# watsonyanghx/GAN_Lib_Tensorflow

Measured on AMD Instinct MI355X. Metric: images/sec (G+D step) SNGAN-ResNet CIFAR-10 bs=64, higher is better.
Workload: dtype bf16; 1 GPU; SNGAN ResNet CIFAR-10 32x32 bs=64 hinge: 1 G update (2x64 fakes) + 5 D updates (64 real + 64 fake) per step; global_batch=64, per_gpu_batch=64, parallelism=dp1, graphs=True, finite=True, collectives_in_graphs=False, grad_wire=fp32

## Files before the change

gan_lib_tensorflow_amd/csrc/conv_igemm.hip:

```cpp
#include "gank_common.h"
#ifdef GANK_TUNING
static __device__ int gank_stats_dbg = 0;
static void gank_stats_dbg_init() {
  static const int v = gank_tune("GANK_STATS_DBG", 0);
  static bool done = false;
  if (!done) { done = true; if (v) (void)hipMemcpyToSymbol(HIP_SYMBOL(gank_stats_dbg), &v, sizeof(int)); }
}
#else
static inline void gank_stats_dbg_init() {}
#endif
#include <stdlib.h>
#include <type_traits>

#ifndef GANK_KMODE
#define GANK_KMODE 0
#endif
#define IG_IN_ZEROINS2X 16
#define IG_IN_STRIDE2 32
#define IG_RES_UP2X 128

struct IgemmArgs {
  const bf16* x;
  const bf16* w;
  const float* bias;
// ... 686 lines not shown
    u32x4 v = {0u, 0u, 0u, 0u};
    if (row < a.Cout && row < 3) v = *reinterpret_cast<const u32x4*>(a.w + (long)row * a.Kpad + c8 * 8);
    *reinterpret_cast<u32x4*>(sW + row * wrow + c8 * 8) = v;
  }

  int h_off[6], h_lds[6];
#pragma unroll
  for (int j = 0; j < 6; j++) {
    const int q = tid + NT * j;
    const int hp = q >> 3, cc = q & 7;
    const int iy = py0 - 1 + hp / 18, ix = px0 - 1 + hp % 18;
    const bool ok = q < PHALO * 8 && (unsigned)iy < (unsigned)a.H && (unsigned)ix < (unsigned)a.W;
    h_off[j] = ok ? (((n * a.H + iy) * a.W + ix) * a.Cin + cc * 8) * 2 : OOB;
    h_lds[j] = (q < PHALO * 8) ? (hp / 18) * HROWP + (hp % 18) * LROW + cc * 8 : -1;
  }
  u32x4 rH[6];
  constexpr bool NORM = (MODE & 8) != 0;
  f32x4 nm[NORM ? 8 : 1];
  const float* np_mu = nullptr;
  const float* np_ga = nullptr;
  const float* np_be = nullptr;
  if constexpr (NORM) {
    int lb = a.cbn_labels[n];
    lb = lb < 0 ? 0 : (lb >= a.cbn_n_labels ? a.cbn_n_labels - 1 : lb);
    np_mu = a.cbn_stats + (long)(n / a.cbn_n_per_group) * 2 * a.Cin + (tid & 7) * 8;
    np_ga = a.cbn_gamma + (long)lb * a.Cin + (tid & 7) * 8;
    np_be = a.cbn_beta + (long)lb * a.Cin + (tid & 7) * 8;
  }
  auto load_halo = [&](int c) {
#pragma unroll
    for (int j = 0; j < 6; j++)
      rH[j] = __builtin_amdgcn_raw_buffer_load_b128(rs_x, h_off[j] == OOB ? OOB : h_off[j] + c * 128, 0, 0);
    if constexpr (NORM) {
      nm[0] = *reinterpret_cast<const f32x4*>(np_mu + c * 64); nm[1] = *reinterpret_cast<const f32x4*>(np_mu + c * 64 + 4);
      nm[2] = *reinterpret_cast<const f32x4*>(np_mu + a.Cin + c * 64); nm[3] = *reinterpret_cast<const f32x4*>(np_mu + a.Cin + c * 64 + 4);
      nm[4] = *reinterpret_cast<const f32x4*>(np_ga + c * 64); nm[5] = *reinterpret_cast<const f32x4*>(np_ga + c * 64 + 4);
      nm[6] = *reinterpret_cast<const f32x4*>(np_be + c * 64); nm[7] = *reinterpret_cast<const f32x4*>(np_be + c * 64 + 4);
    }
  };
  auto store_halo = [&]() {
#pragma unroll
    for (int j = 0; j < 6; j++) {
      if (h_lds[j] >= 0) {
        u32x4 v = rH[j];
        if constexpr (NORM) {
          if (h_off[j] != OOB) {
            const bf16x8 xv = __builtin_bit_cast(bf16x8, v);
            bf16x8 o;
#pragma unroll
            for (int e = 0; e < 8; e++) {
              const float mu = e < 4 ? nm[0][e] : nm[1][e - 4], iv = e < 4 ? nm[2][e] : nm[3][e - 4];
              const float ga = e < 4 ? nm[4][e] : nm[5][e - 4], be = e < 4 ? nm[6][e] : nm[7][e - 4];
              const float t = (bf2f(xv[e]) - mu) * iv * ga + be;
              o[e] = f2bf(fmaxf(t, 0.f));
            }
            v = __builtin_bit_cast(u32x4, o);
          }
        } else if constexpr ((MODE & 1) != 0) {
          v = relu_bf16x8(v);
        }
        *reinterpret_cast<u32x4*>(sP + h_lds[j]) = v;
      }
    }
  };

  f32x16 acc;
#pragma unroll
  for (int e = 0; e < 16; e++) acc[e] = 0.f;
  const int pb = (wave * 2 + (r >> 4) + 1) * HROWP + ((r & 15) + 1) * LROW + h * 8;
  const int ab = (r < 3 ? r : 3) * wrow + h * 8;

  const int nchunks = a.Cin >> 6;
  load_halo(0);
  store_halo();
  __syncthreads();
#pragma unroll 1
  for (int c = 0; c < nchunks; c++) {
    if (c + 1 < nchunks) load_halo(c + 1);
    const bf16* pW = sW + ab + c * 64;
#pragma unroll
    for (int tap = 0; tap < 9; tap++) {
      const int toff = (tap / 3 - 1) * HROWP + (tap % 3 - 1) * LROW;
#pragma unroll
      for (int kk = 0; kk < 4; kk++) {
        const bf16x8 fa = *reinterpret_cast<const bf16x8*>(pW + tap * a.Cin + kk * 16);
        const bf16x8 fb = *reinterpret_cast<const bf16x8*>(sP + pb + toff + kk * 16);
        acc = GANK_MFMA32(fa, fb, acc);
      }
    }
    if (c + 1 < nchunks) {
      __syncthreads();
      store_halo();
      __syncthreads();
    }
  }

  if (h == 0) {
    const bool otanh = (a.flags & GANK_OUT_TANH) != 0;
    const int py = wave * 2 + (r >> 4), px = r & 15;
    const long m = ((long)(n * a.H + py0 + py)) * a.W + px0 + px;
#pragma unroll
    for (int e = 0; e < 3; e++) {
      if (e >= a.Cout) break;
      float t = acc[e] * a.scale;
      if (a.bias) t += a.bias[e];
      if (a.mask) t = (bf2f(a.mask[m * a.Cout + e]) > 0.f) ? t : 0.f;
      if (a.res) t += bf2f(a.res[m * a.Cout + e]);
      a.y[m * a.Cout + e] = f2bf(otanh ? tanhf(t) : t);
    }
  }
}

template <int MODE>
static int launch_few(const IgemmArgs& a0, hipStream_t s) {
  IgemmArgs a = a0;
  a.tiles_m = a.N * (a.H / 8) * (a.W / 16);
  a.tiles_n = 1;
  const size_t lds = ((size_t)10 * HROWP + (size_t)4 * (a.Kpad + 8)) * sizeof(bf16);
  auto kern = conv3x3_few_kernel<MODE>;
  GANK_MAX_DYNAMIC_LDS(kern, (int)lds, "conv3x3_few");
  static const std::string tag = gank_format("conv3x3_few_kernel<%d>", MODE);
  gank_prof_tag(0, tag.c_str());
  hipLaunchKernelGGL(kern, dim3(a.tiles_m), dim3(256), lds, s, a);
  GANK_LAUNCH_OK("conv3x3_few");
  return 0;
}
static bool few_ok(const IgemmArgs& a) {
  static const int env = gank_tune("GANK_IGEMM_FEW", 1);
  return env && a.korder == 0 && a.Cout <= 3 && a.CoutPad == 32 && a.Cin % 64 == 0 && a.Kpad == 9 * a.Cin && !(a.flags & IG_RES_UP2X) &&
         (size_t)(10 * HROWP + 4 * (a.Kpad + 8)) * sizeof(bf16) <= 160 * 1024;
}

template <int MODE>
static int launch_patch_phase(const IgemmArgs& a0, hipStream_t s) {
  IgemmArgs a = a0;
  a.tiles_pp = a.N * (a.H / 8) * (a.W / 16);
  a.phase_inner = phase_inner_env();
  a.tiles_m = 4 * a.tiles_pp;
  a.tiles_n = a.CoutPad / 128;
  const size_t lds = ((size_t)10 * HROWP + (size_t)2 * 128 * LROW) * sizeof(bf16);
  auto kern = conv_igemm_patch_kernel<MODE, 128>;
  GANK_MAX_DYNAMIC_LDS(kern, (int)lds, "conv_igemm_patch");
  static const std::string tag = gank_format("conv_igemm_patch_kernel<%d, 128>", MODE);
  gank_prof_tag(0, tag.c_str());
  hipLaunchKernelGGL(kern, dim3(a.tiles_m * a.tiles_n), dim3(256), lds, s, a);
  GANK_LAUNCH_OK("conv_igemm_patch_phase");
  return 0;
}
static bool patch_phase_ok(const IgemmArgs& a) {
  static const int env = gank_tune("GANK_IGEMM_PATCH_PHASE", 1);
  return env && a.W % 16 == 0 && a.H % 8 == 0 && a.CoutPad % 128 == 0 && a.Cout % 4 == 0 && a.Cin % 64 == 0;
}

constexpr int NARROW_LDS = 4 * 32 * 272;
template <int KS, int CIN, bool POOL>
__device__ __forceinline__ void narrow_in_body(const IgemmArgs& a, const int block, char* s_t) {
  constexpr int TAPS = KS * KS, KTOT = TAPS * CIN, PAD = (KS - 1) / 2;
  static_assert(KTOT <= 32, "one 32-deep K-step");
  static_assert(!POOL || KS == 1, "pooled gather: 1x1 only");
  const int lane = threadIdx.x & 63, wave = threadIdx.x >> 6;
  const int r = lane & 31, h = lane >> 5;
  const int tile_n = block % a.tiles_n, tile_m = block / a.tiles_n;
  const int m = tile_m * 128 + wave * 32 + r;
  const bool inrelu = (a.flags & GANK_IN_RELU) != 0;

  int n = 0, oh = 0, ow = 0;
  if (m < a.M) pix_decomp(m, a.H, a.W, a.shw, a.sw, n, oh, ow);
  bf16x8 fb[2];
#pragma unroll
  for (int kk = 0; kk < 2; kk++) {
#pragma unroll
    for (int j = 0; j < 8; j++) {
      const int k = kk * 16 + 8 * h + j;
      const int tap = k / CIN, c = k - tap * CIN;
      const int ih = oh + tap / KS - PAD, iw = ow + tap % KS - PAD;
      const bool ok = m < a.M && k < KTOT && (unsigned)ih < (unsigned)a.H && (unsigned)iw < (unsigned)a.W;
      float val;
      if constexpr (POOL) {
        const int rs = 2 * a.W * CIN;
        const int idx = ok ? ((n * 2 * a.H + 2 * ih) * 2 * a.W + 2 * iw) * CIN + c : 0;
        val = bf2f(f2bf((bf2f(a.x[idx]) + bf2f(a.x[idx + rs]) + bf2f(a.x[idx + CIN]) + bf2f(a.x[idx + rs + CIN])) * 0.25f));
      } else {
        const int idx = ok ? ((n * a.H + ih) * a.W + iw) * CIN + c : 0;
        val = bf2f(a.x[idx]);
      }
      val = ok ? val : 0.f;
      if (inrelu) val = fmaxf(val, 0.f);
      fb[kk][j] = f2bf(val);
    }
  }
  if constexpr (POOL) {
    if (a.aux_out && tile_n == 0 && h == 0 && m < a.M) {
#pragma unroll
      for (int j = 0; j < CIN; j++) a.aux_out[(long)m * CIN + j] = fb[0][j];
    }
  }
  f32x16 acc[4];
#pragma unroll
  for (int i = 0; i < 4; i++)
#pragma unroll
    for (int e = 0; e < 16; e++) acc[i][e] = 0.f;
#pragma unroll
  for (int i = 0; i < 4; i++) {
    const bf16* wr = a.w + (long)(tile_n * 128 + i * 32 + r) * a.Kpad + h * 8;
#pragma unroll
    for (int kk = 0; kk < 2; kk++) {
      const bf16x8 fa = *reinterpret_cast<const bf16x8*>(wr + kk * 16);
      acc[i] = GANK_MFMA32(fa, fb[kk], acc[i]);
    }
  }
  const bool otanh = (a.flags & GANK_OUT_TANH) != 0;
  if (a.korder == 0 && !a.mask && !a.res && !otanh && (a.Cout & 127) == 0) {
    char* mine = s_t + wave * 32 * 272;
#pragma unroll
    for (int i = 0; i < 4; i++) {
      const int ct = tile_n * 128 + i * 32;
#pragma unroll
      for (int q = 0; q < 2; q++) {
        float v[8];
        acc_widen(acc[i], q, a.scale, v);
        bf16x8 o;
        if (a.bias) {
          const f32x4 b0 = *reinterpret_cast<const f32x4*>(a.bias + ct + 16 * q + 8 * h), b1 = *reinterpret_cast<const f32x4*>(a.bias + ct + 16 * q + 8 * h + 4);
#pragma unroll
          for (int e = 0; e < 4; e++) { v[e] += b0[e]; v[4 + e] += b1[e]; }
        }
#pragma unroll
        for (int e = 0; e < 8; e++) o[e] = f2bf(v[e]);
        *reinterpret_cast<bf16x8*>(mine + r * 272 + (i * 32 + 16 * q + 8 * h) * 2) = o;
      }
    }
    asm volatile("s_waitcnt lgkmcnt(0)" ::: "memory");
    const int m_w = tile_m * 128 + wave * 32;
#pragma unroll
    for (int it = 0; it < 8; it++) {
      const int p = it * 4 + (lane >> 4), c16 = lane & 15;
      const u32x4 v = *reinterpret_cast<const u32x4*>(mine + p * 272 + c16 * 16);
      if (m_w + p < a.M) *reinterpret_cast<u32x4*>(a.y + (long)(m_w + p) * a.Cout + tile_n * 128 + c16 * 8) = v;
    }
    return;
  }
  if ((a.Cout & 31) == 0) {
    if (m < a.M) {
#pragma unroll
      for (int i = 0; i < 4; i++) {
        const int ct = tile_n * 128 + i * 32;
        if (ct < a.Cout)
          epi_tile_wide<false>(acc[i], a.scale, a.bias ? a.bias + ct : nullptr, a.mask ? a.mask + (long)m * a.Cout + ct : nullptr,
                               a.res ? a.res + (long)m * a.Cout + ct : nullptr, a.y + (long)m * a.Cout + ct, h, otanh, nullptr);
      }
    }
    return;
  }
#pragma unroll
  for (int i = 0; i < 4; i++) {
    const int co0 = tile_n * 128 + i * 32 + 4 * h;
#pragma unroll
    for (int g = 0; g < 4; g++) {
      const int co = co0 + 8 * g;
      float v[4];
#pragma unroll
      for (int e = 0; e < 4; e++) v[e] = acc[i][4 * g + e] * a.scale;
      if (m < a.M && co < a.Cout) {
        const long o = (long)m * a.Cout + co;
        if (a.bias) {
          const f32x4 b = *reinterpret_cast<const f32x4*>(a.bias + co);
#pragma unroll
          for (int e = 0; e < 4; e++) v[e] += b[e];
        }
        if (a.mask) {
          const bf16x4 mk = *reinterpret_cast<const bf16x4*>(a.mask + o);
#pragma unroll
          for (int e = 0; e < 4; e++) v[e] = (bf2f(mk[e]) > 0.f) ? v[e] : 0.f;
        }
        if (a.res) {
          const bf16x4 rs = *reinterpret_cast<const bf16x4*>(a.res + o);
#pragma unroll
          for (int e = 0; e < 4; e++) v[e] += bf2f(rs[e]);
        }
        bf16x4 out;
#pragma unroll
        for (int e = 0; e < 4; e++) out[e] = f2bf(otanh ? tanhf(v[e]) : v[e]);
        *reinterpret_cast<bf16x4*>(a.y + o) = out;
      }
    }
  }
}

template <int KS, int CIN, bool POOL = false>
__global__ __launch_bounds__(256) void conv_narrow_in_kernel(IgemmArgs a) {
  __shared__ __attribute__((aligned(16))) char s_t[NARROW_LDS];
  narrow_in_body<KS, CIN, POOL>(a, blockIdx.x, s_t);
}
__global__ __launch_bounds__(256) void conv_narrow_in_pair_kernel(IgemmArgs a, IgemmArgs b, int blocks_a) {
  __shared__ __attribute__((aligned(16))) char s_t[NARROW_LDS];
  if ((int)blockIdx.x < blocks_a) narrow_in_body<3, 3, false>(a, blockIdx.x, s_t);
  else narrow_in_body<1, 3, true>(b, blockIdx.x - blocks_a, s_t);
}

template <int KS, int CIN, bool POOL = false>
static int launch_narrow_in(const IgemmArgs& a0, hipStream_t s) {
  IgemmArgs a = a0;
  a.tiles_m = cdiv(a.M, 128);
  a.tiles_n = a.CoutPad / 128;
  static const std::string tag = gank_format("conv_narrow_in_kernel<%d, %d%s>", KS, CIN, POOL ? ", pool" : "");
  gank_prof_tag(0, tag.c_str());
  hipLaunchKernelGGL((conv_narrow_in_kernel<KS, CIN, POOL>), dim3(a.tiles_m * a.tiles_n), dim3(256), 0, s, a);
  GANK_LAUNCH_OK("conv_narrow_in");
  return 0;
}

constexpr int PP_HALO_BYTES = 24576;
constexpr int PP_WSLOT_BYTES = 16384;
constexpr int PP_NSLOT = 6, PP_PD = 4;
constexpr int PP_WRING = 2 * PP_HALO_BYTES;
constexpr int PP_LDS_BYTES = PP_WRING + PP_NSLOT * PP_WSLOT_BYTES;

template <int N>
__device__ __forceinline__ void pp_wait_vmcnt() {
  static_assert(N == 0 || N == 4 || N == 6 || N == 7, "vmcnt value not instantiated");
  if constexpr (N == 0) asm volatile("s_waitcnt vmcnt(0)" ::: "memory");
  if constexpr (N == 4) asm volatile("s_waitcnt vmcnt(4)" ::: "memory");
  if constexpr (N == 6) asm volatile("s_waitcnt vmcnt(6)" ::: "memory");
  if constexpr (N == 7) asm volatile("s_waitcnt vmcnt(7)" ::: "memory");
}

#ifndef GANK_PP_M16
#define GANK_PP_M16 1
#endif
#ifdef GANK_ACT_F16
#define GANK_MFMA16(a, b, c) __builtin_amdgcn_mfma_f32_16x16x32_f16(a, b, c, 0, 0, 0)
#else
#define GANK_MFMA16(a, b, c) __builtin_amdgcn_mfma_f32_16x16x32_bf16(a, b, c, 0, 0, 0)
#endif
template <int MODE, int PW, bool STATS = false>
__global__ __launch_bounds__(512) void conv_igemm_pp_kernel(IgemmArgs a) {
  constexpr bool PHASE = (MODE & 4) != 0;
  constexpr int NT = PHASE ? 4 : 9;
  constexpr int PHH = 256 / PW;
  constexpr int HW_ = PW + 2, HROW = HW_ * 64;
  constexpr int HPX = (PHH + 2) * HW_;
  constexpr int RS = 32 / PW;
  constexpr int HSW = PW == 16 ? 1 : 2;
#if GANK_PP_M16
  auto pp_hswz = [](int hx) { return (hx >> 1) & 2; };
  auto pp_wswz = [](int co) { return (co >> 1) & 2; };
#else
  auto pp_hswz = [](int hx) { return (hx >> HSW) & 3; };
  auto pp_wswz = [](int co) { return (co >> 2) & 3; };
#endif
  static_assert(PW == 32 || PW == 16, "patch width");
  static_assert(HPX * 64 <= PP_HALO_BYTES, "halo image");
  extern __shared__ __attribute__((aligned(16))) char smem[];
  typedef __attribute__((address_space(3))) void* lds_t;
  const int tid = threadIdx.x, lane = tid & 63;
  const int wave = __builtin_amdgcn_readfirstlane(tid >> 6);
  const int wm = wave >> 2, wn = wave & 3;
  const int r = lane & 31, h = lane >> 5;
  const int prow = RS == 1 ? 0 : (r >> 4), pcol = RS == 1 ? r : (r & 15);

  const int nwg = a.tiles_m * a.tiles_n;
  const int lid = xcd_remap(blockIdx.x, nwg);
  const int tile_n = lid % a.tiles_n;
  int tile_m = lid / a.tiles_n;
  int phase = 0;
  if constexpr (PHASE) {
    if (a.phase_inner) { phase = tile_m & 3; tile_m >>= 2; }
    else { phase = tile_m / a.tiles_pp; tile_m -= phase * a.tiles_pp; }
  }
  const int pad_h = PHASE ? 1 - (phase >> 1) : 1, pad_w = PHASE ? 1 - (phase & 1) : 1;
  const int pw = a.W / PW, ph = a.H / PHH;
  const int n = tile_m / (pw * ph), pr = tile_m - n * pw * ph;
  const int py0 = (pr / pw) * PHH, px0 = (pr % pw) * PW;

  constexpr unsigned OOB = 0x7FFFFFF0u;
  const __amdgpu_buffer_rsrc_t rs_x = __builtin_amdgcn_make_buffer_rsrc(const_cast<bf16*>(a.x), 0, a.N * a.H * a.W * a.Cin * 2, 0x00020000);
  const __amdgpu_buffer_rsrc_t rs_w = __builtin_amdgcn_make_buffer_rsrc(const_cast<bf16*>(a.w) + (PHASE ? (long)phase * a.CoutPad * a.Kpad : 0L), 0,
                                                                        a.CoutPad * a.Kpad * 2, 0x00020000);

  unsigned h_off[6];
#pragma unroll
  for (int j = 0; j < 6; j++) {
    const int q = (j * 4 + wn) * 64 + lane;
    const int hp = q >> 2, hy = hp / HW_, hx = hp - hy * HW_;
    const int iy = py0 - 1 + hy, ix = px0 - 1 + hx;
    const bool ok = hp < HPX && (unsigned)iy < (unsigned)a.H && (unsigned)ix < (unsigned)a.W;
    h_off[j] = ok ? (unsigned)((((n * a.H + iy) * a.W + ix) * a.Cin + (((q & 3) ^ pp_hswz(hx)) << 3)) * 2) : OOB;
  }
  int w_off[2];
#pragma unroll
  for (int j = 0; j < 2; j++) {
    const int q = (j * 8 + wave) * 64 + lane;
    const int co = q >> 2;
    w_off[j] = ((tile_n * 256 + co) * a.Kpad + (((q & 3) ^ pp_wswz(co)) << 3)) * 2;
  }
  constexpr int ND = PHASE ? 2 : 3;
#if GANK_PP_M16
  const int p16 = lane & 15, kc = lane >> 4;
  constexpr int RPT = PW / 16;
  int a_lane, b_lane[ND];
  a_lane = PP_WRING + (wn * 64 + p16) * 64 + ((kc ^ pp_wswz(p16)) << 4);
#pragma unroll
  for (int d = 0; d < ND; d++) {
    const int hx = p16 + d + (PHASE ? 1 - pad_w : 0);
    const int hy = wm * (PHH / 2) + (PHASE ? 1 - pad_h : 0);
    b_lane[d] = hy * HROW + hx * 64 + ((kc ^ pp_hswz(hx)) << 4);
  }
#else
  int a_lane[2], b_lane[ND][2];
#pragma unroll
  for (int kk = 0; kk < 2; kk++) {
    a_lane[kk] = PP_WRING + (wn * 64 + r) * 64 + (((kk * 2 + h) ^ pp_wswz(r)) << 4);
#pragma unroll
    for (int d = 0; d < ND; d++) {
      const int hx = pcol + d + (PHASE ? 1 - pad_w : 0);
      const int hy = wm * (PHH / 2) + prow + (PHASE ? 1 - pad_h : 0);
      b_lane[d][kk] = hy * HROW + hx * 64 + (((kk * 2 + h) ^ pp_hswz(hx)) << 4);
    }
  }
#endif

  const int nch = a.Cin >> 5;
  auto issue_w = [&](int slot_bytes, int c, int tap) {
    const int koff = (tap * a.Cin + c * 32) * 2;
#pragma unroll
    for (int j = 0; j < 2; j++)
      __builtin_amdgcn_raw_ptr_buffer_load_lds(rs_w, (lds_t)(smem + PP_WRING + slot_bytes + (j * 8 + wave) * 1024), 16, w_off[j], koff, 0, 0);
  };
  auto issue_h = [&](int buf, int c, int j0) {
#pragma unroll
    for (int j = j0; j < j0 + 3; j++)
      __builtin_amdgcn_raw_ptr_buffer_load_lds(rs_x, (lds_t)(smem + buf * PP_HALO_BYTES + (j * 4 + wn) * 1024), 16, (int)(h_off[j] + (unsigned)c * 64u), 0, 0, 0);
  };

#if GANK_PP_M16
  f32x4 acc[4][8];
#pragma unroll
  for (int i = 0; i < 4; i++)
#pragma unroll
    for (int j = 0; j < 8; j++) acc[i][j] = f32x4{0.f, 0.f, 0.f, 0.f};
#else
  f32x16 acc[2][4];
#pragma unroll
  for (int i = 0; i < 2; i++)
#pragma unroll
    for (int j = 0; j < 4; j++)
#pragma unroll
      for (int e = 0; e < 16; e++) acc[i][j][e] = 0.f;
#endif

  if (wm == 1) { issue_h(0, 0, 0); issue_h(0, 0, 3); }
  {
    int c = 0, t = 0;
#pragma unroll
    for (int q = 0; q < PP_PD; q++) {
      issue_w(q * PP_WSLOT_BYTES, c, t);
      if (++t == NT) { t = 0; c++; }
      if (c >= nch) { c = nch - 1; t = NT - 1; }
    }
  }
// ... 415 lines not shown
  const bool pp_ok = pp_env() && patch_geom && a.Cout % 256 == 0 && a.Kpad == a.taps * a.Cin && pp_enough_blocks(a, 1) &&
                     (pp_env() >= 2 || pp_patch_width(a.H, a.W) == 32);
  if (narrow_ok) {
    rc = a.ks == 3 ? launch_narrow_in<3, 3>(a, s) : launch_narrow_in<1, 3>(a, s);
  } else if (pp_ok) {
    const bool relu = (a.flags & GANK_IN_RELU) != 0;
    if (pp_patch_width(a.H, a.W) == 32) rc = relu ? launch_pp<1, 32>(a, s) : launch_pp<0, 32>(a, s);
    else rc = relu ? launch_pp<1, 16>(a, s) : launch_pp<0, 16>(a, s);
  } else if (patch_ok) {
    rc = (a.flags & GANK_IN_RELU) ? launch_patch<1, 128>(a, s) : launch_patch<0, 128>(a, s);
  } else if (patch32_ok && few_ok(a)) {
    rc = (a.flags & GANK_IN_RELU) ? launch_few<1>(a, s) : launch_few<0>(a, s);
  } else if (patch32_ok) {
    rc = (a.flags & GANK_IN_RELU) ? launch_patch<1, 32>(a, s) : launch_patch<0, 32>(a, s);
  } else if (packed) {
    if (a.CoutPad % 64 == 0) rc = launch_cfg<2, 2, 1, 1, true, 1, 0>(a, s);
    else rc = launch_cfg<4, 1, 2, 1, true, 1, 0>(a, s);
#ifdef GANK_TUNING
  } else if (a.CoutPad % 128 == 0 && tiles128 >= t128_min() && pf_env >= 20) {
    if (pf_env == 20) rc = launch_mode<4, 2, 2, 2, 1>(a, s);
    else if (pf_env == 22 && a.CoutPad % 256 == 0) rc = launch_mode<2, 4, 2, 2, 2>(a, s);
    else if (pf_env == 23 && a.CoutPad % 256 == 0) rc = launch_mode<4, 2, 2, 4, 2>(a, s);
    else rc = launch_mode<4, 2, 2, 2, 2>(a, s);
  } else if (a.CoutPad % 128 == 0 && tiles128 >= t128_min() && (pf_env == 1 || pf_env == 3)) {
    rc = pf_env == 1 ? launch_mode<2, 2, 2, 2, 1>(a, s) : launch_mode<2, 2, 2, 2, 3>(a, s);
  } else if (a.CoutPad % 64 == 0 && !(a.CoutPad % 128 == 0 && tiles128 >= t128_min()) && (pf_env == 1 || pf_env == 11 || pf_env == 12 || pf_env == 3)) {
    rc = (pf_env == 1 || pf_env == 11) ? launch_mode<2, 2, 1, 1, 1>(a, s) : launch_mode<2, 2, 1, 1, 2>(a, s);
#endif
  } else if (a.CoutPad % 128 == 0 && tiles128 >= t128_min()) {
    rc = launch_mode<2, 2, 2, 2, 2>(a, s);
  } else if (a.CoutPad % 64 == 0) {
    rc = launch_mode<2, 2, 1, 1, 4>(a, s);
  } else {
    rc = launch_mode<4, 1, 2, 1, 2>(a, s);
  }
  gank_prof_end(0, s);
  return rc;
}

static int stats_setup(IgemmArgs& a, float* stat_sums, int groups, int N, int Cout, hipStream_t s, int flags) {
  tl_stats_done = 0;
  if (!stat_sums) return 0;
  gank_stats_dbg_init();
  a.stat_prezeroed = (flags & GANK_STATS_PREZEROED) != 0;
  GANK_REQUIRE(groups > 0 && N % groups == 0, "conv statistics: batch %d not divisible by %d towers", N, groups);
  a.stat_sums = stat_sums;
  a.stat_n_per_group = N / groups;
  a.stat_groups = groups;
  return 0;
}
static void stats_zero(const IgemmArgs& a, hipStream_t s) {
  if (a.stat_prezeroed) return;
  const int n = a.stat_groups * GANK_STAT_SLOTS * 2 * a.Cout;
  hipLaunchKernelGGL(ig_zero_kernel, dim3((n + 255) / 256), dim3(256), 0, s, a.stat_sums, n);
}

static int conv2d_fprop_impl(const void* x, const void* wf, const float* bias, const void* residual,
                             const void* relu_ref, void* y, int N, int H, int W, int Cin, int Cout, int ksize,
                             int flags, float scale, float* stat_sums, int groups, void* stream) {
  GANK_REQUIRE(ksize % 2 == 1, "conv2d_fprop: even filter sizes are not on this path (ksize=%d)", ksize);
  GANK_REQUIRE(!(flags & GANK_IN_UPSAMPLE2X) || (H % 2 == 0 && W % 2 == 0), "conv2d_fprop: upsample needs even output size");
  IgemmArgs a{};
  a.x = (const bf16*)x; a.w = (const bf16*)wf; a.bias = bias; a.res = (const bf16*)residual;
  a.mask = (const bf16*)relu_ref; a.y = (bf16*)y;
  a.N = N; a.H = H; a.W = W;
  const bool up = flags & GANK_IN_UPSAMPLE2X;
  a.Hin = up ? H / 2 : H; a.Win = up ? W / 2 : W;
  a.Cin = Cin; a.Cout = Cout; a.ks = ksize; a.pad = (ksize - 1) / 2;
  a.flags = (flags & (GANK_IN_UPSAMPLE2X | GANK_IN_RELU | GANK_OUT_TANH)) |
            ((flags & GANK_RES_UPSAMPLE2X) ? IG_RES_UP2X : 0);
  GANK_REQUIRE(!(flags & GANK_RES_UPSAMPLE2X) || (residual && H % 2 == 0 && W % 2 == 0), "conv2d_fprop: RES_UPSAMPLE2X needs a residual and even output size");
  a.scale = scale;
  if (stats_setup(a, stat_sums, groups, N, Cout, (hipStream_t)stream, flags)) return 1;
  return gank_igemm_dispatch(a, (hipStream_t)stream);
}

extern "C" int gank_conv2d_fprop(const void* x, const void* wf, const float* bias, const void* residual,
                                 const void* relu_ref, void* y, int N, int H, int W, int Cin, int Cout, int ksize,
                                 int flags, float scale, void* stream) {
  return conv2d_fprop_impl(x, wf, bias, residual, relu_ref, y, N, H, W, Cin, Cout, ksize, flags, scale, nullptr, 0, stream);
}
extern "C" int gank_conv2d_fprop_stats(const void* x, const void* wf, const float* bias, const void* residual,
                                       const void* relu_ref, void* y, int N, int H, int W, int Cin, int Cout, int ksize,
                                       int flags, float scale, float* stat_sums, int groups, int* produced, void* stream) {
  GANK_REQUIRE(stat_sums && produced, "conv2d_fprop_stats: null statistics pointers");
  const int rc = conv2d_fprop_impl(x, wf, bias, residual, relu_ref, y, N, H, W, Cin, Cout, ksize, flags, scale, stat_sums, groups, stream);
  *produced = tl_stats_done;
  return rc;
}

extern "C" int gank_cbn_relu_conv3x3_fprop(const void* x, const int32_t* labels, const float* gamma, const float* beta, const float* stats,
                                           const void* wf, const float* bias, void* y, int N, int H, int W, int Cin, int Cout,
                                           int groups, int n_labels, int flags, void* stream) {
  GANK_REQUIRE(x && labels && gamma && beta && stats && wf && y, "cbn_relu_conv3x3_fprop: null pointer");
  GANK_REQUIRE(groups > 0 && N % groups == 0 && n_labels > 0, "cbn_relu_conv3x3_fprop: batch %d / %d towers", N, groups);
  GANK_REQUIRE(Cin % 64 == 0 && W % 16 == 0 && H % 8 == 0, "cbn_relu_conv3x3_fprop: needs Cin %% 64 == 0, W %% 16 == 0, H %% 8 == 0");
  IgemmArgs a{};
  a.x = (const bf16*)x; a.w = (const bf16*)wf; a.bias = bias; a.y = (bf16*)y;
  a.N = N; a.H = H; a.W = W; a.Hin = H; a.Win = W; a.Cin = Cin; a.Cout = Cout; a.ks = 3; a.pad = 1;
  a.flags = flags & GANK_OUT_TANH;
  a.scale = 1.f;
  a.taps = 9; a.CoutPad = roundup(Cout, 32); a.Kpad = roundup(9 * Cin, 64); a.nsteps = a.Kpad / 64;
  a.M = N * H * W; a.sw = log2_or_neg(W); a.shw = log2_or_neg(H * W);
  GANK_REQUIRE(a.CoutPad == 32 || a.CoutPad % 128 == 0, "cbn_relu_conv3x3_fprop: Cout must pad to 32 or a multiple of 128 (got %d)", Cout);
  GANK_REQUIRE((long)N * H * W * Cin < (1L << 30), "cbn_relu_conv3x3_fprop: tensor too large (32-bit byte offsets)");
  a.cbn_stats = stats; a.cbn_gamma = gamma; a.cbn_beta = beta; a.cbn_labels = labels;
  a.cbn_n_per_group = N / groups; a.cbn_n_labels = n_labels;
  hipStream_t s = (hipStream_t)stream;
  gank_prof_begin(0, 2.0 * a.M * (double)Cout * 9 * Cin, s, 2.0 * ((double)a.M * Cin + 9.0 * Cin * Cout + (double)a.M * Cout));
  const int rc = a.CoutPad == 32 ? (few_ok(a) ? launch_few<8>(a, s) : launch_patch<8, 32>(a, s)) : launch_patch<8, 128>(a, s);
  gank_prof_end(0, s);
  return rc;
}

extern "C" int gank_meanpool_conv1x1_fprop(const void* x, const void* wf, const float* bias, void* y, void* pooled,
                                           int N, int H, int W, int Cin, int Cout, void* stream) {
  GANK_REQUIRE(x && wf && y && N > 0 && H > 0 && W > 0, "meanpool_conv1x1_fprop: bad arguments");
  GANK_REQUIRE(Cin == 3, "meanpool_conv1x1_fprop: built for 3-channel images (Cin = %d)", Cin);
  IgemmArgs a{};
  a.x = (const bf16*)x; a.w = (const bf16*)wf; a.bias = bias; a.y = (bf16*)y; a.aux_out = (bf16*)pooled;
  a.N = N; a.H = H; a.W = W; a.Hin = 2 * H; a.Win = 2 * W; a.Cin = Cin; a.Cout = Cout; a.ks = 1; a.pad = 0;
  a.scale = 1.f;
  a.taps = 1; a.CoutPad = roundup(Cout, 32); a.Kpad = roundup(Cin, 64); a.nsteps = a.Kpad / 64;
  a.M = N * H * W; a.sw = log2_or_neg(W); a.shw = log2_or_neg(H * W);
  GANK_REQUIRE(a.CoutPad % 128 == 0 && Cout % 4 == 0, "meanpool_conv1x1_fprop: Cout must be a multiple of 4 that pads to a multiple of 128 (got %d)", Cout);
  GANK_REQUIRE((long)N * 4 * H * W * Cin < (1L << 30), "meanpool_conv1x1_fprop: tensor too large (32-bit offsets)");
  hipStream_t s = (hipStream_t)stream;
  gank_prof_begin(0, 2.0 * a.M * (double)Cout * Cin, s, 2.0 * (4.0 * a.M * Cin + (double)Cin * Cout + (double)a.M * Cout));
  const int rc = launch_narrow_in<1, 3, true>(a, s);
  gank_prof_end(0, s);
  return rc;
}

extern "C" int gank_image_conv_pair_fprop(const void* x, const void* wf1, const float* bias1, void* y1, const void* wfs, const float* biass, void* ys,
                                          void* pooled, int N, int H, int W, int Cout1, int Couts, void* stream) {
  GANK_REQUIRE(x && wf1 && y1 && wfs && ys && N > 0 && H > 0 && W > 0 && H % 2 == 0 && W % 2 == 0, "image_conv_pair_fprop: bad arguments");
  GANK_REQUIRE(Cout1 % 128 == 0 && Couts % 128 == 0, "image_conv_pair_fprop: channel counts must be multiples of 128 (got %d, %d)", Cout1, Couts);
  GANK_REQUIRE((long)N * H * W * 3 < (1L << 30) && (long)N * H * W * Cout1 < (1L << 31), "image_conv_pair_fprop: tensor too large (32-bit offsets)");
  IgemmArgs a{}, b{};
  a.x = (const bf16*)x; a.w = (const bf16*)wf1; a.bias = bias1; a.y = (bf16*)y1;
  a.N = N; a.H = H; a.W = W; a.Hin = H; a.Win = W; a.Cin = 3; a.Cout = Cout1; a.ks = 3; a.pad = 1; a.scale = 1.f;
  a.taps = 9; a.CoutPad = Cout1; a.Kpad = roundup(27, 64); a.nsteps = 1;
  a.M = N * H * W; a.sw = log2_or_neg(W); a.shw = log2_or_neg(H * W);
  a.tiles_m = cdiv(a.M, 128); a.tiles_n = a.CoutPad / 128;
  { static const int ko_env = gank_tune("GANK_IGEMM_KORDER", 0); a.korder = ko_env; }
  const int Hp = H / 2, Wp = W / 2;
  b.x = (const bf16*)x; b.w = (const bf16*)wfs; b.bias = biass; b.y = (bf16*)ys; b.aux_out = (bf16*)pooled;
  b.N = N; b.H = Hp; b.W = Wp; b.Hin = H; b.Win = W; b.Cin = 3; b.Cout = Couts; b.ks = 1; b.pad = 0; b.scale = 1.f;
  b.taps = 1; b.CoutPad = Couts; b.Kpad = roundup(3, 64); b.nsteps = 1;
  b.M = N * Hp * Wp; b.sw = log2_or_neg(Wp); b.shw = log2_or_neg(Hp * Wp);
  b.tiles_m = cdiv(b.M, 128); b.tiles_n = b.CoutPad / 128;
  b.korder = 0;
  hipStream_t s = (hipStream_t)stream;
  const int blocks_a = a.tiles_m * a.tiles_n, blocks_b = b.tiles_m * b.tiles_n;
  gank_prof_begin(0, 2.0 * a.M * (double)Cout1 * 27 + 2.0 * b.M * (double)Couts * 3, s,
                  2.0 * ((double)a.M * 3 + 27.0 * Cout1 + (double)a.M * Cout1 + 3.0 * Couts + (double)b.M * Couts));
  gank_prof_tag(0, "conv_narrow_in_pair_kernel");
  hipLaunchKernelGGL(conv_narrow_in_pair_kernel, dim3(blocks_a + blocks_b), dim3(256), 0, s, a, b, blocks_a);
  gank_prof_end(0, s);
  GANK_LAUNCH_OK("image_conv_pair_fprop");
  return 0;
}

extern "C" int gank_conv2d_dgrad(const void* dy, const void* wd, const void* residual, const void* relu_ref, void* dx,
                                 int N, int H, int W, int Cin, int Cout, int ksize, int flags, float scale, void* stream) {
  GANK_REQUIRE(ksize % 2 == 1, "conv2d_dgrad: even filter sizes are not on this path (ksize=%d)", ksize);
  IgemmArgs a{};
  a.x = (const bf16*)dy; a.w = (const bf16*)wd; a.bias = nullptr; a.res = (const bf16*)residual;
  a.mask = (const bf16*)relu_ref; a.y = (bf16*)dx;
  a.N = N; a.H = H; a.W = W;
  const bool up = flags & GANK_IN_UPSAMPLE2X;
  a.Hin = up ? H / 2 : H; a.Win = up ? W / 2 : W;
  a.Cin = Cout; a.Cout = Cin; a.ks = ksize; a.pad = (ksize - 1) / 2;
  a.flags = (flags & (GANK_IN_UPSAMPLE2X | GANK_IN_RELU));
  a.scale = scale;
  return gank_igemm_dispatch(a, (hipStream_t)stream);
}


extern "C" int gank_conv2d_general_fprop(const void* x, const void* wf, const float* bias, void* y, int N, int Hin, int Win,
                                         int Hout, int Wout, int Cin, int Cout, int ksize, int stride, int pad, int flags, void* stream) {
  GANK_REQUIRE(stride == 1 || stride == 2, "conv2d_general_fprop: stride %d (1 or 2)", stride);
  GANK_REQUIRE(pad >= 0 && pad < ksize, "conv2d_general_fprop: pad %d outside [0, ksize)", pad);
  GANK_REQUIRE(!((flags & GANK_IN_UPSAMPLE2X) && stride == 2), "conv2d_general_fprop: upsampled input with stride 2");
  GANK_REQUIRE(Hin > 0 && Win > 0 && Hout > 0 && Wout > 0, "conv2d_general_fprop: bad sizes");
  IgemmArgs a{};
  a.x = (const bf16*)x; a.w = (const bf16*)wf; a.bias = bias; a.y = (bf16*)y;
  a.N = N; a.H = Hout; a.W = Wout; a.Hin = Hin; a.Win = Win;
  a.Cin = Cin; a.Cout = Cout; a.ks = ksize; a.pad = pad;
  a.flags = (flags & (GANK_IN_UPSAMPLE2X | GANK_IN_RELU | GANK_OUT_TANH)) | (stride == 2 ? IG_IN_STRIDE2 : 0);
  a.scale = 1.f;
  return gank_igemm_dispatch(a, (hipStream_t)stream);
}
extern "C" int gank_conv2d_general_dgrad(const void* dy, const void* wd, const void* relu_ref, void* dx, int N, int Hx, int Wx,
                                         int Hdy, int Wdy, int Cin, int Cout, int ksize, int pad, void* stream) {
  GANK_REQUIRE(pad >= 0 && pad < ksize, "conv2d_general_dgrad: pad %d outside [0, ksize)", pad);
  IgemmArgs a{};
  a.x = (const bf16*)dy; a.w = (const bf16*)wd; a.mask = (const bf16*)relu_ref; a.y = (bf16*)dx;
  a.N = N; a.H = Hx; a.W = Wx; a.Hin = Hdy; a.Win = Wdy;
  a.Cin = Cout; a.Cout = Cin; a.ks = ksize; a.pad = ksize - 1 - pad;
  a.scale = 1.f;
  return gank_igemm_dispatch(a, (hipStream_t)stream);
}

static int upconv3x3_fprop_impl(const void* x, const void* wph, const float* bias, const void* residual, void* y,
                                int N, int Hl, int Wl, int Cin, int Cout, int flags, float* stat_sums, int groups, void* stream) {
  GANK_REQUIRE(Cin % 64 == 0, "upconv3x3_fprop: Cin must be a multiple of 64 (got %d)", Cin);
  IgemmArgs a{};
  a.x = (const bf16*)x; a.w = (const bf16*)wph; a.bias = bias; a.res = (const bf16*)residual; a.y = (bf16*)y;
  a.N = N; a.H = Hl; a.W = Wl; a.Hin = Hl; a.Win = Wl;
  a.Cin = Cin; a.Cout = Cout; a.ks = 2; a.pad = 0;
  a.flags = flags & GANK_OUT_TANH;
  a.scale = 1.f;
  hipStream_t s = (hipStream_t)stream;
  a.taps = 4; a.CoutPad = roundup(Cout, 32); a.Kpad = 4 * Cin; a.nsteps = a.Kpad / 64;
  a.M = N * Hl * Wl; a.sw = log2_or_neg(Wl); a.shw = log2_or_neg(Hl * Wl);
  GANK_REQUIRE((long)N * Hl * Wl * Cin < (1L << 30) && (long)a.M * 4 * Cout < (1L << 31), "upconv3x3_fprop: tensor too large");
  if (stats_setup(a, stat_sums, groups, N, Cout, s, flags)) return 1;
  gank_prof_begin(0, 2.0 * a.M * 4.0 * (double)Cout * 4 * Cin, s, 2.0 * ((double)a.M * Cin + 16.0 * Cin * Cout + 4.0 * a.M * Cout + (residual ? 4.0 * a.M * Cout : 0.0)));
  int rc;
  const long tiles128 = 4L * cdiv(a.M, 128) * (a.CoutPad / 128);
  if (pp_phase_ok(a)) rc = launch_pp_phase(a, s);
  else if (patch_phase_ok(a)) rc = launch_patch_phase<4>(a, s);
  else if (a.CoutPad % 128 == 0 && tiles128 >= t128_min()) rc = launch_phase<2, 2, 2, 2, 2>(a, s);
  else if (a.CoutPad % 64 == 0) rc = launch_phase<2, 2, 1, 1, 4>(a, s);
  else rc = launch_phase<4, 1, 2, 1, 2>(a, s);
  gank_prof_end(0, s);
  return rc;
}

extern "C" int gank_upconv3x3_fprop(const void* x, const void* wph, const float* bias, const void* residual, void* y,
                                    int N, int Hl, int Wl, int Cin, int Cout, int flags, void* stream) {
  return upconv3x3_fprop_impl(x, wph, bias, residual, y, N, Hl, Wl, Cin, Cout, flags, nullptr, 0, stream);
}
extern "C" int gank_upconv3x3_fprop_stats(const void* x, const void* wph, const float* bias, const void* residual, void* y,
                                          int N, int Hl, int Wl, int Cin, int Cout, int flags, float* stat_sums, int groups, int* produced,
                                          void* stream) {
  GANK_REQUIRE(stat_sums && produced, "upconv3x3_fprop_stats: null statistics pointers");
  const int rc = upconv3x3_fprop_impl(x, wph, bias, residual, y, N, Hl, Wl, Cin, Cout, flags, stat_sums, groups, stream);
  *produced = tl_stats_done;
  return rc;
}

extern "C" int gank_upconv3x3_dgrad(const void* dy, const void* wd4, const void* relu_ref, void* dx, int N, int Hl, int Wl,
                                    int Cin, int Cout, void* stream) {
  IgemmArgs a{};
  a.x = (const bf16*)dy; a.w = (const bf16*)wd4; a.mask = (const bf16*)relu_ref; a.y = (bf16*)dx;
  a.N = N; a.H = Hl; a.W = Wl; a.Hin = 2 * Hl; a.Win = 2 * Wl;
  a.Cin = Cout; a.Cout = Cin; a.ks = 4; a.pad = 1;
  a.flags = IG_IN_STRIDE2;
  a.scale = 1.f;
  return gank_igemm_dispatch(a, (hipStream_t)stream);
}

extern "C" int gank_convpool3x3_fprop(const void* x, const void* wp4, const float* bias, const void* residual, void* y,
                                      int N, int Hp, int Wp, int Cin, int Cout, int flags, void* stream) {
  IgemmArgs a{};
  a.x = (const bf16*)x; a.w = (const bf16*)wp4; a.bias = bias; a.res = (const bf16*)residual; a.y = (bf16*)y;
  a.N = N; a.H = Hp; a.W = Wp; a.Hin = 2 * Hp; a.Win = 2 * Wp;
  a.Cin = Cin; a.Cout = Cout; a.ks = 4; a.pad = 1;
  a.flags = IG_IN_STRIDE2 | (flags & GANK_IN_RELU);
  a.scale = 1.f;
  return gank_igemm_dispatch(a, (hipStream_t)stream);
}

extern "C" int gank_convpool3x3_dgrad(const void* dy, const void* wphd, const void* relu_ref, void* dx, int N, int Hp, int Wp,
                                      int Cin, int Cout, void* stream) {
  GANK_REQUIRE(Cout % 64 == 0, "convpool3x3_dgrad: Cout must be a multiple of 64 (got %d)", Cout);
  IgemmArgs a{};
  a.x = (const bf16*)dy; a.w = (const bf16*)wphd; a.mask = (const bf16*)relu_ref; a.y = (bf16*)dx;
  a.N = N; a.H = Hp; a.W = Wp; a.Hin = Hp; a.Win = Wp;
  a.Cin = Cout; a.Cout = Cin; a.ks = 2; a.pad = 0;
  a.flags = 0;
  a.scale = 1.f;
  hipStream_t s = (hipStream_t)stream;
  a.taps = 4; a.CoutPad = roundup(Cin, 32); a.Kpad = 4 * Cout; a.nsteps = a.Kpad / 64;
  a.M = N * Hp * Wp; a.sw = log2_or_neg(Wp); a.shw = log2_or_neg(Hp * Wp);
  GANK_REQUIRE((long)N * Hp * Wp * Cout < (1L << 30) && (long)a.M * 4 * Cin < (1L << 31), "convpool3x3_dgrad: tensor too large");
  gank_prof_begin(0, 2.0 * a.M * 4.0 * (double)Cin * 4 * Cout, s, 2.0 * ((double)a.M * Cout + 16.0 * Cin * Cout + 4.0 * a.M * Cin + (relu_ref ? 4.0 * a.M * Cin : 0.0)));
  int rc;
  const long tiles128 = 4L * cdiv(a.M, 128) * (a.CoutPad / 128);
  if (pp_phase_ok(a)) rc = launch_pp_phase(a, s);
  else if (patch_phase_ok(a)) rc = launch_patch_phase<4>(a, s);
  else if (a.CoutPad % 128 == 0 && tiles128 >= t128_min()) rc = launch_phase<2, 2, 2, 2, 2>(a, s);
  else if (a.CoutPad % 64 == 0) rc = launch_phase<2, 2, 1, 1, 4>(a, s);
  else rc = launch_phase<4, 1, 2, 1, 2>(a, s);
  gank_prof_end(0, s);
  return rc;
}

static int deconv_pad_before(int ks) { int t = ks - 2; if (t < 0) t = 0; return t / 2; }

extern "C" int gank_deconv2d_fprop(const void* x, const void* wz, const float* bias, void* y, int N, int H, int W,
                                   int Cin, int Cout, int ksize, void* stream) {
  IgemmArgs a{};
  a.x = (const bf16*)x; a.w = (const bf16*)wz; a.bias = bias; a.y = (bf16*)y;
  a.N = N; a.H = 2 * H; a.W = 2 * W; a.Hin = H; a.Win = W;
  a.Cin = Cin; a.Cout = Cout; a.ks = ksize;
  a.pad = ksize - 1 - deconv_pad_before(ksize);
  a.flags = IG_IN_ZEROINS2X;
  a.scale = 1.f;
  return gank_igemm_dispatch(a, (hipStream_t)stream);
}

extern "C" int gank_deconv2d_dgrad(const void* dy, const void* wfz, void* dx, int N, int H, int W, int Cin, int Cout,
                                   int ksize, void* stream) {
  IgemmArgs a{};
  a.x = (const bf16*)dy; a.w = (const bf16*)wfz; a.y = (bf16*)dx;
  a.N = N; a.H = H; a.W = W; a.Hin = 2 * H; a.Win = 2 * W;
  a.Cin = Cout; a.Cout = Cin; a.ks = ksize; a.pad = deconv_pad_before(ksize);
  a.flags = IG_IN_STRIDE2;
// ... 4 lines not shown
```

Before: 58340 images/sec.

## Make narrow-input conv kernels persistent with prefetched gathers and hoisted weights

```diff
diff --git a/gan_lib_tensorflow_amd/csrc/conv_igemm.hip b/gan_lib_tensorflow_amd/csrc/conv_igemm.hip
--- a/gan_lib_tensorflow_amd/csrc/conv_igemm.hip
+++ b/gan_lib_tensorflow_amd/csrc/conv_igemm.hip
@@ -862,79 +862,146 @@
   return env && a.W % 16 == 0 && a.H % 8 == 0 && a.CoutPad % 128 == 0 && a.Cout % 4 == 0 && a.Cin % 64 == 0;
 }
 
-constexpr int NARROW_LDS = 4 * 32 * 272;
+#ifndef NARROW_WAVES
+#define NARROW_WAVES 2
+#endif
+constexpr int NARROW_T_LDS = 4 * 32 * 272;
+constexpr int NARROW_LDS = NARROW_T_LDS + 4 * 128 * 4;
+
 template <int KS, int CIN, bool POOL>
-__device__ __forceinline__ void narrow_in_body(const IgemmArgs& a, const int block, char* s_t) {
-  constexpr int TAPS = KS * KS, KTOT = TAPS * CIN, PAD = (KS - 1) / 2;
+struct NarrowGather {
+  static constexpr int TAPS = KS * KS, KTOT = TAPS * CIN, PAD = (KS - 1) / 2, NRAW = POOL ? 4 : 1;
   static_assert(KTOT <= 32, "one 32-deep K-step");
   static_assert(!POOL || KS == 1, "pooled gather: 1x1 only");
+  bf16 raw[NRAW][16];
+  unsigned ok;
+
+  __device__ __forceinline__ void issue(const IgemmArgs& a, const int m, const int h) {
+    int n = 0, oh = 0, ow = 0;
+    if (m < a.M) pix_decomp(m, a.H, a.W, a.shw, a.sw, n, oh, ow);
+    int pix = (POOL ? (n * 2 * a.H + 2 * oh) * 2 * a.W + 2 * ow : (n * a.H + oh) * a.W + ow) * CIN;
+    asm volatile("" : "+v"(pix));
+    const int row = a.W * CIN;
+    ok = 0u;
+#pragma unroll
+    for (int kk = 0; kk < 2; kk++) {
+#pragma unroll
+      for (int j = 0; j < 8; j++) {
+        const int k0 = kk * 16 + j, k1 = k0 + 8;
+        const int dy0 = (k0 / CIN) / KS - PAD, dx0 = (k0 / CIN) % KS - PAD, dy1 = (k1 / CIN) / KS - PAD, dx1 = (k1 / CIN) % KS - PAD;
+        const int off0 = dy0 * row + dx0 * CIN + k0 % CIN, off1 = dy1 * row + dx1 * CIN + k1 % CIN;
+        const int dy = h ? dy1 : dy0, dx = h ? dx1 : dx0;
+        const bool kin = h ? k1 < KTOT : k0 < KTOT;
+        const bool in = m < a.M && kin && (unsigned)(oh + dy) < (unsigned)a.H && (unsigned)(ow + dx) < (unsigned)a.W;
+        ok |= in ? (1u << (kk * 8 + j)) : 0u;
+        const int idx = in ? pix + (h ? off1 : off0) : 0;
+        const char* xb = reinterpret_cast<const char*>(a.x);
+        raw[0][kk * 8 + j] = *reinterpret_cast<const bf16*>(xb + (unsigned)(2 * idx));
+        if constexpr (POOL) {
+          raw[1][kk * 8 + j] = *reinterpret_cast<const bf16*>(xb + (unsigned)(2 * (idx + 2 * row)));
+          raw[2][kk * 8 + j] = *reinterpret_cast<const bf16*>(xb + (unsigned)(2 * (idx + CIN)));
+          raw[3][kk * 8 + j] = *reinterpret_cast<const bf16*>(xb + (unsigned)(2 * (idx + 2 * row + CIN)));
+        }
+      }
+    }
+  }
+  __device__ __forceinline__ void finish(const bool inrelu, bf16x8 (&fb)[2]) const {
+#pragma unroll
+    for (int kk = 0; kk < 2; kk++) {
+#pragma unroll
+      for (int j = 0; j < 8; j++) {
+        const int e = kk * 8 + j;
+        float val;
+        if constexpr (POOL) val = bf2f(f2bf((bf2f(raw[0][e]) + bf2f(raw[1][e]) + bf2f(raw[2][e]) + bf2f(raw[3][e])) * 0.25f));
+        else val = bf2f(raw[0][e]);
+        val = ((ok >> e) & 1u) ? val : 0.f;
+        if (inrelu) val = fmaxf(val, 0.f);
+        fb[kk][j] = f2bf(val);
+      }
+    }
+  }
+};
+
+__device__ __forceinline__ bool narrow_in_fast(const IgemmArgs& a) {
+  return a.korder == 0 && !a.mask && !a.res && !(a.flags & GANK_OUT_TANH) && (a.Cout & 127) == 0;
+}
+template <bool FAST>
+__device__ __forceinline__ void narrow_in_epilogue(const IgemmArgs& a, const f32x16 (&acc)[4], int tile_m, int tile_n, int m, int wave, int lane,
+                                                   bool otanh, char* mine, const float* bias_w);
+
+template <int KS, int CIN, bool POOL, bool FAST>
+__device__ __forceinline__ void narrow_in_tiles(const IgemmArgs& a, const int u_first, const int stride, char* s_t) {
   const int lane = threadIdx.x & 63, wave = threadIdx.x >> 6;
   const int r = lane & 31, h = lane >> 5;
-  const int tile_n = block % a.tiles_n, tile_m = block / a.tiles_n;
-  const int m = tile_m * 128 + wave * 32 + r;
-  const bool inrelu = (a.flags & GANK_IN_RELU) != 0;
-
-  int n = 0, oh = 0, ow = 0;
-  if (m < a.M) pix_decomp(m, a.H, a.W, a.shw, a.sw, n, oh, ow);
-  bf16x8 fb[2];
-#pragma unroll
-  for (int kk = 0; kk < 2; kk++) {
-#pragma unroll
-    for (int j = 0; j < 8; j++) {
-      const int k = kk * 16 + 8 * h + j;
-      const int tap = k / CIN, c = k - tap * CIN;
-      const int ih = oh + tap / KS - PAD, iw = ow + tap % KS - PAD;
-      const bool ok = m < a.M && k < KTOT && (unsigned)ih < (unsigned)a.H && (unsigned)iw < (unsigned)a.W;
-      float val;
-      if constexpr (POOL) {
-        const int rs = 2 * a.W * CIN;
-        const int idx = ok ? ((n * 2 * a.H + 2 * ih) * 2 * a.W + 2 * iw) * CIN + c : 0;
-        val = bf2f(f2bf((bf2f(a.x[idx]) + bf2f(a.x[idx + rs]) + bf2f(a.x[idx + CIN]) + bf2f(a.x[idx + rs + CIN])) * 0.25f));
-      } else {
-        const int idx = ok ? ((n * a.H + ih) * a.W + iw) * CIN + c : 0;
-        val = bf2f(a.x[idx]);
-      }
-      val = ok ? val : 0.f;
-      if (inrelu) val = fmaxf(val, 0.f);
-      fb[kk][j] = f2bf(val);
-    }
-  }
-  if constexpr (POOL) {
-    if (a.aux_out && tile_n == 0 && h == 0 && m < a.M) {
-#pragma unroll
-      for (int j = 0; j < CIN; j++) a.aux_out[(long)m * CIN + j] = fb[0][j];
-    }
-  }
-  f32x16 acc[4];
-#pragma unroll
-  for (int i = 0; i < 4; i++)
-#pragma unroll
-    for (int e = 0; e < 16; e++) acc[i][e] = 0.f;
+  const int tile_n = u_first % a.tiles_n, stride_m = stride >= a.tiles_n ? stride / a.tiles_n : 1;
+  int tile_m = u_first / a.tiles_n;
+  const bool inrelu = (a.flags & GANK_IN_RELU) != 0, otanh = (a.flags & GANK_OUT_TANH) != 0;
+
+  bf16x8 fa[4][2];
 #pragma unroll
   for (int i = 0; i < 4; i++) {
     const bf16* wr = a.w + (long)(tile_n * 128 + i * 32 + r) * a.Kpad + h * 8;
 #pragma unroll
-    for (int kk = 0; kk < 2; kk++) {
-      const bf16x8 fa = *reinterpret_cast<const bf16x8*>(wr + kk * 16);
-      acc[i] = GANK_MFMA32(fa, fb[kk], acc[i]);
-    }
-  }
-  const bool otanh = (a.flags & GANK_OUT_TANH) != 0;
-  if (a.korder == 0 && !a.mask && !a.res && !otanh && (a.Cout & 127) == 0) {
-    char* mine = s_t + wave * 32 * 272;
+    for (int kk = 0; kk < 2; kk++) fa[i][kk] = *reinterpret_cast<const bf16x8*>(wr + kk * 16);
+  }
+  u32x2 bias2 = {0x80000000u, 0x80000000u};
+  if (FAST && a.bias) bias2 = *reinterpret_cast<const u32x2*>(a.bias + tile_n * 128 + 2 * lane);
+  NarrowGather<KS, CIN, POOL> g;
+  g.issue(a, tile_m * 128 + wave * 32 + r, h);
+  char* mine = s_t + wave * 32 * 272;
+  float* bias_w = reinterpret_cast<float*>(s_t + NARROW_T_LDS) + wave * 128;
+  if (FAST) *reinterpret_cast<u32x2*>(bias_w + 2 * lane) = bias2;
+  bf16x8 fb[2];
+  g.finish(inrelu, fb);
+
+  for (;;) {
+    const int next_m = tile_m + stride_m;
+    const bool more = next_m < a.tiles_m;
+    if (more) g.issue(a, next_m * 128 + wave * 32 + r, h);
+    const int m = tile_m * 128 + wave * 32 + r;
+    if constexpr (POOL) {
+      if (a.aux_out && tile_n == 0 && h == 0 && m < a.M) {
+#pragma unroll
+        for (int j = 0; j < CIN; j++) a.aux_out[(long)m * CIN + j] = fb[0][j];
+      }
+    }
+    f32x16 acc[4];
+#pragma unroll
+    for (int i = 0; i < 4; i++)
+#pragma unroll
+      for (int e = 0; e < 16; e++) acc[i][e] = 0.f;
+#pragma unroll
+    for (int i = 0; i < 4; i++)
+#pragma unroll
+      for (int kk = 0; kk < 2; kk++) acc[i] = GANK_MFMA32(fa[i][kk], fb[kk], acc[i]);
+    narrow_in_epilogue<FAST>(a, acc, tile_m, tile_n, m, wave, lane, otanh, mine, bias_w);
+    if (!more) break;
+    g.finish(inrelu, fb);
+    tile_m = next_m;
+  }
+}
+template <int KS, int CIN, bool POOL>
+__device__ __forceinline__ void narrow_in_body(const IgemmArgs& a, const int u_first, const int stride, char* s_t) {
+  if (u_first >= a.tiles_m * a.tiles_n) return;
+  if (narrow_in_fast(a)) narrow_in_tiles<KS, CIN, POOL, true>(a, u_first, stride, s_t);
+  else narrow_in_tiles<KS, CIN, POOL, false>(a, u_first, stride, s_t);
+}
+
+template <bool FAST>
+__device__ __forceinline__ void narrow_in_epilogue(const IgemmArgs& a, const f32x16 (&acc)[4], const int tile_m, const int tile_n, const int m,
+                                                   const int wave, const int lane, const bool otanh, char* mine, const float* bias_w) {
+  const int r = lane & 31, h = lane >> 5;
+  if constexpr (FAST) {
 #pragma unroll
     for (int i = 0; i < 4; i++) {
-      const int ct = tile_n * 128 + i * 32;
 #pragma unroll
       for (int q = 0; q < 2; q++) {
         float v[8];
         acc_widen(acc[i], q, a.scale, v);
         bf16x8 o;
-        if (a.bias) {
-          const f32x4 b0 = *reinterpret_cast<const f32x4*>(a.bias + ct + 16 * q + 8 * h), b1 = *reinterpret_cast<const f32x4*>(a.bias + ct + 16 * q + 8 * h + 4);
-#pragma unroll
-          for (int e = 0; e < 4; e++) { v[e] += b0[e]; v[4 + e] += b1[e]; }
-        }
+        const f32x4 b0 = *reinterpret_cast<const f32x4*>(bias_w + i * 32 + 16 * q + 8 * h), b1 = *reinterpret_cast<const f32x4*>(bias_w + i * 32 + 16 * q + 8 * h + 4);
+#pragma unroll
+        for (int e = 0; e < 4; e++) { v[e] += b0[e]; v[4 + e] += b1[e]; }
 #pragma unroll
         for (int e = 0; e < 8; e++) o[e] = f2bf(v[e]);
         *reinterpret_cast<bf16x8*>(mine + r * 272 + (i * 32 + 16 * q + 8 * h) * 2) = o;
@@ -942,12 +1009,16 @@
     }
     asm volatile("s_waitcnt lgkmcnt(0)" ::: "memory");
     const int m_w = tile_m * 128 + wave * 32;
+    const int p0 = lane >> 4, c16 = lane & 15;
+    u32x4 t[8];
+#pragma unroll
+    for (int it = 0; it < 8; it++) t[it] = *reinterpret_cast<const u32x4*>(mine + (it * 4 + p0) * 272 + c16 * 16);
 #pragma unroll
     for (int it = 0; it < 8; it++) {
-      const int p = it * 4 + (lane >> 4), c16 = lane & 15;
-      const u32x4 v = *reinterpret_cast<const u32x4*>(mine + p * 272 + c16 * 16);
-      if (m_w + p < a.M) *reinterpret_cast<u32x4*>(a.y + (long)(m_w + p) * a.Cout + tile_n * 128 + c16 * 8) = v;
-    }
+      const int p = it * 4 + p0;
+      if (m_w + p < a.M) *reinterpret_cast<u32x4*>(a.y + (long)(m_w + p) * a.Cout + tile_n * 128 + c16 * 8) = t[it];
+    }
+    asm volatile("s_waitcnt lgkmcnt(0)" ::: "memory");
     return;
   }
   if ((a.Cout & 31) == 0) {
@@ -998,14 +1069,41 @@
 }
 
 template <int KS, int CIN, bool POOL = false>
-__global__ __launch_bounds__(256) void conv_narrow_in_kernel(IgemmArgs a) {
+__global__ __launch_bounds__(256, NARROW_WAVES) void conv_narrow_in_kernel(IgemmArgs a) {
   __shared__ __attribute__((aligned(16))) char s_t[NARROW_LDS];
-  narrow_in_body<KS, CIN, POOL>(a, blockIdx.x, s_t);
-}
-__global__ __launch_bounds__(256) void conv_narrow_in_pair_kernel(IgemmArgs a, IgemmArgs b, int blocks_a) {
+  narrow_in_body<KS, CIN, POOL>(a, blockIdx.x, gridDim.x, s_t);
+}
+__global__ __launch_bounds__(256, NARROW_WAVES) void conv_narrow_in_pair_kernel(IgemmArgs a, IgemmArgs b, int blocks_a) {
   __shared__ __attribute__((aligned(16))) char s_t[NARROW_LDS];
-  if ((int)blockIdx.x < blocks_a) narrow_in_body<3, 3, false>(a, blockIdx.x, s_t);
-  else narrow_in_body<1, 3, true>(b, blockIdx.x - blocks_a, s_t);
+  const int j = blockIdx.x, grid = gridDim.x;
+  if (blocks_a > 0) {
+    if (j < blocks_a) narrow_in_body<3, 3, false>(a, j, blocks_a, s_t);
+    else narrow_in_body<1, 3, true>(b, j - blocks_a, grid - blocks_a, s_t);
+    return;
+  }
+  const int units_a = a.tiles_m * a.tiles_n;
+  narrow_in_body<3, 3, false>(a, j, grid, s_t);
+  const int i = (units_a - j + grid - 1) / grid;
+  narrow_in_body<1, 3, true>(b, j + i * grid - units_a, grid, s_t);
+}
+
+static int narrow_cu_count() {
+  static const int n = [] {
+    int dev = 0;
+    hipDeviceProp_t p;
+    if (hipGetDevice(&dev) != hipSuccess || hipGetDeviceProperties(&p, dev) != hipSuccess || p.multiProcessorCount <= 0) return 256;
+    return (int)p.multiProcessorCount;
+  }();
+  return n;
+}
+static int narrow_grid(int units, int mult) {
+  static const int persist = gank_tune("GANK_NARROW_PERSIST", 1);
+  static const int k = gank_tune("GANK_NARROW_K", 2);
+  if (!persist) return units;
+  long cap = (long)k * narrow_cu_count();
+  cap -= cap % mult;
+  if (cap < mult) cap = mult;
+  return units <= cap ? units : (int)cap;
 }
 
 template <int KS, int CIN, bool POOL = false>
@@ -1015,7 +1113,7 @@
   a.tiles_n = a.CoutPad / 128;
   static const std::string tag = gank_format("conv_narrow_in_kernel<%d, %d%s>", KS, CIN, POOL ? ", pool" : "");
   gank_prof_tag(0, tag.c_str());
-  hipLaunchKernelGGL((conv_narrow_in_kernel<KS, CIN, POOL>), dim3(a.tiles_m * a.tiles_n), dim3(256), 0, s, a);
+  hipLaunchKernelGGL((conv_narrow_in_kernel<KS, CIN, POOL>), dim3(narrow_grid(a.tiles_m * a.tiles_n, a.tiles_n)), dim3(256), 0, s, a);
   GANK_LAUNCH_OK("conv_narrow_in");
   return 0;
 }
@@ -1737,11 +1835,13 @@
   b.tiles_m = cdiv(b.M, 128); b.tiles_n = b.CoutPad / 128;
   b.korder = 0;
   hipStream_t s = (hipStream_t)stream;
-  const int blocks_a = a.tiles_m * a.tiles_n, blocks_b = b.tiles_m * b.tiles_n;
+  const int units_a = a.tiles_m * a.tiles_n, units_b = b.tiles_m * b.tiles_n;
+  const int grid = narrow_grid(units_a + units_b, a.tiles_n * b.tiles_n);
+  const int blocks_a = grid == units_a + units_b ? units_a : 0;
   gank_prof_begin(0, 2.0 * a.M * (double)Cout1 * 27 + 2.0 * b.M * (double)Couts * 3, s,
                   2.0 * ((double)a.M * 3 + 27.0 * Cout1 + (double)a.M * Cout1 + 3.0 * Couts + (double)b.M * Couts));
   gank_prof_tag(0, "conv_narrow_in_pair_kernel");
-  hipLaunchKernelGGL(conv_narrow_in_pair_kernel, dim3(blocks_a + blocks_b), dim3(256), 0, s, a, b, blocks_a);
+  hipLaunchKernelGGL(conv_narrow_in_pair_kernel, dim3(grid), dim3(256), 0, s, a, b, blocks_a);
   gank_prof_end(0, s);
   GANK_LAUNCH_OK("image_conv_pair_fprop");
   return 0;
```

Result: no change. 58650 images/sec, median of 6 (+0.5%).
